# innnky/vispeech

Hardware: AMD Instinct MI355X
Metric: 44.1kHz samples/sec (higher is better)
Workload: dtype f32 (split-f16 MFMA, 3-term); 1 GPU; C3: 64 mixed zh/ja utterances (~5 s each) per GPU, 44.1 kHz, hop 512, phoneme/duration/F0/energy/noise supplied, random-init (synthetic) weights of configs/config.json; 2 batches in flight per GPU; utterances_per_gpu=64, global_batch=64, padded_frames=489, frames_padded=31296, frames_computed=28902, parallelism=shard1, generator=f16s, controls=all, batches_in_flight=2

## Files before the change

### include/vispeech_hip.h

```cpp
#ifndef VISPEECH_HIP_H
#define VISPEECH_HIP_H

#include <stdint.h>

#ifdef __cplusplus
extern "C" {
#endif

#define VSP_ABI_VERSION 7

enum {
  VSP_OK = 0,
  VSP_ERR_ARG = -1,
  VSP_ERR_STATE = -2,
  VSP_ERR_HIP = -3,
  VSP_ERR_KEY = -4,
  VSP_ERR_SHAPE = -5,
  VSP_ERR_WORKSPACE = -6,
  VSP_ERR_UNSUPPORTED = -7
};

#define VSP_MAX_LIST 8

typedef struct vsp_config {
// ... 91 lines not shown
int64_t vsp_flow_workspace_bytes(const vsp_ctx* ctx, int B, int Tf);
int vsp_flow_reverse(vsp_ctx* ctx, void* stream, int B, int Tf, const float* z_p, const float* g,
                     const int64_t* frame_lengths, float* z, void* workspace, int64_t workspace_bytes);
int64_t vsp_wn_layer_workspace_bytes(const vsp_ctx* ctx, int which, int B, int T);
int vsp_wn_layer(vsp_ctx* ctx, void* stream, int which, int layer, int B, int T, float* x, const float* g,
                 const int64_t* lengths, float* skip, int accumulate, void* workspace, int64_t workspace_bytes);
int64_t vsp_generator_workspace_bytes(const vsp_ctx* ctx, int B, int T);
int vsp_generator_kind(const vsp_ctx* ctx);
int vsp_generator(vsp_ctx* ctx, void* stream, int B, int T, const float* z, const float* g,
                  float* o, void* workspace, int64_t workspace_bytes);
int vsp_generator_ragged(vsp_ctx* ctx, void* stream, int B, int T, const float* z, const float* g,
                         const int64_t* lengths, float* o, void* workspace, int64_t workspace_bytes);

int vsp_generator_halo_frames(const vsp_ctx* ctx);
int vsp_generator_frame_dependence(const vsp_ctx* ctx, int* back, int* fwd);
int64_t vsp_generator_stream_workspace_bytes(const vsp_ctx* ctx, int B, int chunk_frames);
int vsp_generator_stream_chunk(vsp_ctx* ctx, void* stream, int B, int T, const float* z, const float* g, int f0, int f1,
                               float* o_chunk, void* workspace, int64_t workspace_bytes);

typedef struct vsp_stream_row {
  const float* z;
  int64_t z_channel_stride;
  const float* g;
  int32_t L, f0, f1;
} vsp_stream_row;
int vsp_stream_rows_plan(const vsp_ctx* ctx, int B, const vsp_stream_row* rows, int32_t* lo, int32_t* hi, int32_t* span_max);
int64_t vsp_generator_stream_rows_workspace_bytes(const vsp_ctx* ctx, int B, int chunk_frames);
int vsp_generator_stream_rows(vsp_ctx* ctx, void* stream, int B, const vsp_stream_row* rows, void* out, int64_t out_stride,
                              int pcm, void* workspace, int64_t workspace_bytes);

// ... 173 lines not shown
```

### vispeech_amd/_lib.py

```python
from __future__ import annotations

import ctypes as C
import os
from typing import Optional

_HERE = os.path.dirname(os.path.abspath(__file__))
LIB_PATH = os.environ.get("VSP_LIB_PATH") or os.path.join(_HERE, "lib", "libvispeech_hip.so")

VSP_MAX_LIST = 8
ABI_VERSION = 7
DTYPES = {"float32": 0, "float16": 1, "bfloat16": 2, "float64": 3}
PROF_GENERATOR, PROF_ATTENTION, PROF_FRAME = 0, 1, 2
FLAG_NONFINITE_LATENT, FLAG_NONFINITE_WAVE = 1, 2

ERRORS = {0: "VSP_OK", -1: "VSP_ERR_ARG", -2: "VSP_ERR_STATE", -3: "VSP_ERR_HIP", -4: "VSP_ERR_KEY",
          -5: "VSP_ERR_SHAPE", -6: "VSP_ERR_WORKSPACE", -7: "VSP_ERR_UNSUPPORTED"}


class VspConfig(C.Structure):
    _fields_ = [
        ("n_vocab", C.c_int32), ("inter_channels", C.c_int32), ("hidden_channels", C.c_int32),
        ("filter_channels", C.c_int32), ("n_heads", C.c_int32), ("n_layers", C.c_int32),
        ("kernel_size", C.c_int32), ("n_resblock_kernels", C.c_int32),
        ("resblock_kernel_sizes", C.c_int32 * VSP_MAX_LIST), ("n_resblock_dilations", C.c_int32),
# ... 89 lines not shown
    "vsp_set_isolated": (_I, [_P, _I]),
    "vsp_get_isolated": (_I, [_P]),
    "vsp_set_noise_seeds": (_I, [_P, C.POINTER(_U64), _I]),
    "vsp_set_row_controls": (_I, [_P, C.POINTER(VspRowControl), _I]),
    "vsp_encoder_workspace_bytes": (_I64, [_P, _I, _I]),
    "vsp_encoder": (_I, [_P, _P, _I, _I, _I, _P, _P, _P, _P, _I64]),
    "vsp_length_regulate": (_I, [_P, _P, _I, _I, _I, _I, _P, _P, _P]),
    "vsp_flow_workspace_bytes": (_I64, [_P, _I, _I]),
    "vsp_flow_reverse": (_I, [_P, _P, _I, _I, _P, _P, _P, _P, _P, _I64]),
    "vsp_generator_workspace_bytes": (_I64, [_P, _I, _I]),
    "vsp_generator": (_I, [_P, _P, _I, _I, _P, _P, _P, _P, _I64]),
    "vsp_generator_ragged": (_I, [_P, _P, _I, _I, _P, _P, _P, _P, _P, _I64]),
    "vsp_generator_kind": (_I, [_P]),
    "vsp_generator_halo_frames": (_I, [_P]),
    "vsp_generator_frame_dependence": (_I, [_P, C.POINTER(_I), C.POINTER(_I)]),
    "vsp_generator_stream_workspace_bytes": (_I64, [_P, _I, _I]),
    "vsp_generator_stream_chunk": (_I, [_P, _P, _I, _I, _P, _P, _I, _I, _P, _P, _I64]),
    "vsp_stream_rows_plan": (_I, [_P, _I, C.POINTER(VspStreamRow), C.POINTER(C.c_int32), C.POINTER(C.c_int32),
                                  C.POINTER(C.c_int32)]),
    "vsp_generator_stream_rows_workspace_bytes": (_I64, [_P, _I, _I]),
    "vsp_generator_stream_rows": (_I, [_P, _P, _I, C.POINTER(VspStreamRow), _P, _I64, _I, _P, _I64]),
    "vsp_stream_rows_output_plan": (_I, [_I, _I, _I, _I, _I, C.POINTER(VspStreamRow), C.POINTER(_I64), C.POINTER(_I64),
                                         C.POINTER(_I64), C.POINTER(_I64)]),
    "vsp_output_history_samples": (_I, [_I, _I, _I]),
    "vsp_stream_rows_out_samples": (_I64, [_I, _I, _I, _I, _I]),
    "vsp_generator_stream_rows_output": (_I, [_P, _P, _I, C.POINTER(VspStreamRowOut), _P, _I64, _I, _P, _I64]),
    "vsp_flow_forward": (_I, [_P, _P, _I, _I, _P, _P, _P, _P, _P, _I64]),
    "vsp_voice_conversion_workspace_bytes": (_I64, [_P, _I, _I]),
    "vsp_voice_conversion": (_I, [_P, _P, _I, _I, _P, _P, _P, _P, _P, _P, _P, _P, _P, _P, _P, _P, _P, _I64]),
    "vsp_posterior_workspace_bytes": (_I64, [_P, _I, _I]),
# ... 132 lines not shown
```

### vispeech_amd/csrc/api_common.h

```cpp
#pragma once
#include <algorithm>
#include <cmath>
#include <cstdlib>
#include <cstring>
#include <vector>

#include "model.h"
#include "row_controls.h"

namespace vsp {

struct T3 {
  float* p = nullptr;
  long bs = 0, cs = 0;
  T3 chan(int c) const { return T3{p ? p + (size_t)c * cs : nullptr, bs, cs}; }
};

struct Ws {
  char* base;
  size_t cap;
  size_t cur = 0;
  bool dry;
  bool overflow = false;
  Ws(void* b, size_t c, bool d) : base((char*)b), cap(c), dry(d) {}
// ... 202 lines not shown
  return ctx->fail(VSP_ERR_WORKSPACE, "%s workspace too small: %lld < %lld bytes", what, (long long)workspace_bytes, (long long)need);
}

int check_ready(vsp_ctx* ctx);
int check_vc(vsp_ctx* ctx);

void run_encoder_masked(Run& r, const EncoderW& E, int B, int T, T3 x_in, const int64_t* lengths, T3 y_out);
void mask3(Run& r, T3 x, const int64_t* lengths, int B, int C, int T);
void run_wn(Run& r, const Conv* cond, const std::vector<Conv>& in, const std::vector<Conv>& res, const std::vector<Conv>& skip,
            int nl, int B, int T, T3 H, T3 ACT, T3 OUT, float* gc, long gc_bs, const float* g, const int64_t* lengths);
void run_flow(Run& r, int B, int T, T3 z, const float* g, const int64_t* lengths, bool reverse = true);
void run_posterior(Run& r, int B, int T, T3 y, const int64_t* lengths, const float* g, const float* noise, T3 Z, T3 M, T3 LOGS,
                   float noise_scale = 1.f);
void draw_noise_rows(Run& r, uint64_t* seeds_dev, const int64_t* lengths, int B, int C, int T, float* drawn);
void run_gen(Run& r, int B, int T, T3 z, const int64_t* in_lengths, const float* g, float* o);

}
```

### vispeech_amd/csrc/api_context.hip

```cpp
#include "api_common.h"

using namespace vsp;

namespace vsp {

int check_ready(vsp_ctx* ctx) {
  if (!ctx) return VSP_ERR_ARG;
  if (!ctx->ready) return ctx->fail(VSP_ERR_STATE, "weights not finalised");
  return VSP_OK;
}

int check_vc(vsp_ctx* ctx) {
  const int rc = check_ready(ctx);
  if (rc) return rc;
  if (ctx->cfg.spec_channels <= 0) return ctx->fail(VSP_ERR_STATE, "context was created without spec_channels");
  if (!ctx->model.has_vc) return ctx->fail(VSP_ERR_STATE, "enc_q.* tensors were not loaded before vsp_finalize_weights");
  return VSP_OK;
}

}

extern "C" {

int vsp_abi_version(void) { return VSP_ABI_VERSION; }
// ... 11 lines not shown
  if (const char* e = getenv("VSP_ATT")) ctx->att_f16s = strcmp(e, "f32") != 0;
  bool want_f16 = false;
  if (const char* e = getenv("VSP_GENERATOR")) {
    if (!strcmp(e, "f32")) ctx->gen_mode = 0;
    want_f16 = !strcmp(e, "f16");
  }
  if (const char* e = getenv("VSP_FUSE_PAIRS")) ctx->fuse_pairs = atoi(e) != 0;
  if (const char* e = getenv("VSP_RB2_FUSE")) ctx->rb2_fuse = atoi(e) != 0;
  if (const char* e = getenv("VSP_TIMG")) ctx->t_img = atoi(e) != 0;
  if (const char* e = getenv("VSP_PP")) ctx->pp_pairs = atoi(e) != 0;
  if (const char* e = getenv("VSP_PAIR")) ctx->pair_ring = !strcmp(e, "ring");
  if (const char* e = getenv("VSP_CHAIN_RING")) ctx->chain_ring = atoi(e) != 0;
  if (const char* e = getenv("VSP_CHAIN")) ctx->chain_mask = atoi(e);
  if (const char* e = getenv("VSP_RW64")) ctx->rw64 = atoi(e) != 0;
  if (const char* e = getenv("VSP_TRIM_TAILS")) ctx->trim_tails = atoi(e) != 0;
  if (const char* e = getenv("VSP_COLS")) ctx->cols = atoi(e) != 0;
  if (const char* e = getenv("VSP_COLS_BLOCKS")) ctx->cols_blocks = atol(e);
  if (const char* e = getenv("VSP_COLS_MIN_BLOCKS")) ctx->cols_min_blocks = atol(e);
  if (const char* e = getenv("VSP_ACT_SCALE_LOG2")) {
    const int l = atoi(e);
    ctx->act_scale = std::ldexp(1.f, l < 0 ? 0 : l > 8 ? 8 : l);
  }
  if (const char* e = getenv("VSP_EARLY_FL")) ctx->early_fl = atoi(e) != 0;
  if (const char* e = getenv("VSP_RB_STREAMS")) ctx->rb_streams = atoi(e);
#ifdef VSP_EXPERIMENTS
  if (const char* e = getenv("VSP_ATT_KSPLIT")) ctx->att_ksplit = atoi(e);
  if (const char* e = getenv("VSP_CHUNK_MB")) ctx->chunk_mb = atof(e);
  if (const char* e = getenv("VSP_CHAIN_CH")) ctx->chain_ch = atoi(e);
  if (const char* e = getenv("VSP_CHAIN128")) ctx->chain128_mask = atoi(e);
#endif
// ... 2 lines not shown
  if (want_f16 && ctx->gen_mode == 1) ctx->gen_mode = 2;
  *out = ctx;
  return rc;
}

int vsp_destroy(vsp_ctx* ctx) {
  if (!ctx) return VSP_ERR_ARG;
  for (auto e : ctx->ev_pool) (void)hipEventDestroy(e);
  for (auto e : ctx->sync_ev) (void)hipEventDestroy(e);
  if (ctx->fl_ev) (void)hipEventDestroy(ctx->fl_ev);
  if (ctx->fl_pinned) (void)hipHostFree(ctx->fl_pinned);
  if (ctx->flags_host) (void)hipHostFree(ctx->flags_host);
  for (auto st : ctx->side) if (st) (void)hipStreamDestroy(st);
  if (ctx->arena && ctx->arena_owned) (void)hipFree(ctx->arena);
  if (ctx->out_tab) (void)hipFree(ctx->out_tab);
  for (auto& r : ctx->in_rates) if (r.tab) (void)hipFree(r.tab);
  for (auto& r : ctx->out_rates) if (r.tab) (void)hipFree(r.tab);
  delete ctx;
  return VSP_OK;
}

const char* vsp_last_error(const vsp_ctx* ctx) { return ctx ? ctx->err.c_str() : "null context"; }

int vsp_status(vsp_ctx* ctx, unsigned* flags, int clear) {
  if (!ctx || !flags) return VSP_ERR_ARG;
  *flags = 0u;
  if (!ctx->flags_host) return VSP_OK;
  volatile unsigned* w = ctx->flags_host;
  *flags = clear ? __atomic_exchange_n(ctx->flags_host, 0u, __ATOMIC_ACQ_REL) : *w;
  return VSP_OK;
}

int vsp_begin_weights(vsp_ctx* ctx) {
  if (!ctx) return VSP_ERR_ARG;
  ctx->raw.clear();
  ctx->ready = false;
  ctx->adopted_pending = false;
  return VSP_OK;
}

int vsp_set_weight(vsp_ctx* ctx, const char* key, const float* host_data, const int64_t* shape, int ndim) {
  if (!ctx || !key || !host_data || !shape || ndim < 0 || ndim > 8) return ctx ? ctx->fail(VSP_ERR_ARG, "null argument") : VSP_ERR_ARG;
  const std::string k(key);
  if (k.rfind("enc_q.", 0) == 0 && ctx->cfg.spec_channels <= 0) return VSP_OK;
  auto it = ctx->schema.find(k);
  bool folded_form = false;
  if (it == ctx->schema.end()) {
    auto iv = ctx->schema.find(k + "_v");
    if (iv == ctx->schema.end()) return ctx->fail(VSP_ERR_KEY, "unknown state_dict key '%s'", key);
    it = iv;
    folded_form = true;
  }
// ... 137 lines not shown

int vsp_finalize_weights(vsp_ctx* ctx, void* dev_arena) {
  if (!ctx) return VSP_ERR_ARG;
  if (ctx->model.total_floats == 0) return ctx->fail(VSP_ERR_STATE, "context was not planned (vsp_create failed)");
  const int miss = vsp_missing_weights(ctx);
  if (miss) return ctx->fail(VSP_ERR_STATE, "%d infer-path tensors missing", miss);
  std::vector<float> host;
  int rc = fill_model(ctx, host);
  if (rc) return rc;
  {
    const uint64_t tf = ctx->model.total_floats;
    const uint32_t hdr[6] = {ARENA_MAGIC, (uint32_t)VSP_ABI_VERSION, (uint32_t)(tf & 0xffffffffu), (uint32_t)(tf >> 32),
                             ctx->model.has_vc ? ARENA_FLAG_VC : 0u, config_hash(ctx)};
    std::memcpy(host.data(), hdr, sizeof hdr);
  }
  rc = set_arena(ctx, dev_arena);
  if (rc) return rc;
  hipError_t e = hipMemcpy(ctx->arena, host.data(), host.size() * sizeof(float), hipMemcpyHostToDevice);
  if (e != hipSuccess) return ctx->fail(VSP_ERR_HIP, "hipMemcpy(weight arena): %s", hipGetErrorString(e));
  ctx->adopted_pending = false;
  ctx->ready = true;
  return VSP_OK;
}

int vsp_adopt_packed_weights(vsp_ctx* ctx, void* dev_arena) {
  if (!ctx || !dev_arena) return ctx ? ctx->fail(VSP_ERR_ARG, "null arena") : VSP_ERR_ARG;
  if (ctx->model.total_floats == 0) return ctx->fail(VSP_ERR_STATE, "context was not planned");
  const int rc = set_arena(ctx, dev_arena);
  if (rc) return rc;
  ctx->model.has_vc = false;
  ctx->ready = false;
  ctx->adopted_pending = true;
  return VSP_OK;
}

int vsp_commit_adopted_weights(vsp_ctx* ctx, void* stream) {
  if (!ctx) return VSP_ERR_ARG;
  if (!ctx->adopted_pending || !ctx->arena) return ctx->fail(VSP_ERR_STATE, "no adopted arena to commit");
  uint32_t hdr[6] = {0, 0, 0, 0, 0, 0};
  hipError_t e = hipMemcpyAsync(hdr, ctx->arena, sizeof hdr, hipMemcpyDeviceToHost, (hipStream_t)stream);
  if (e == hipSuccess) e = hipStreamSynchronize((hipStream_t)stream);
  if (e != hipSuccess) return ctx->fail(VSP_ERR_HIP, "arena header read: %s", hipGetErrorString(e));
  const uint64_t tf = (uint64_t)hdr[2] | ((uint64_t)hdr[3] << 32);
  if (hdr[0] != ARENA_MAGIC) return ctx->fail(VSP_ERR_STATE, "adopted arena has no header (bytes not broadcast yet, or not a packed arena)");
  if (hdr[1] != (uint32_t)VSP_ABI_VERSION) return ctx->fail(VSP_ERR_STATE, "adopted arena was packed by ABI %u, this library is ABI %d", hdr[1], VSP_ABI_VERSION);
  if (tf != ctx->model.total_floats || hdr[5] != config_hash(ctx))
    return ctx->fail(VSP_ERR_STATE, "adopted arena was packed for a different configuration");
  ctx->model.has_vc = (hdr[4] & ARENA_FLAG_VC) != 0;
  ctx->adopted_pending = false;
  ctx->ready = true;
  return VSP_OK;
}

int vsp_has_voice_conversion(const vsp_ctx* ctx) { return ctx && ctx->ready && ctx->model.has_vc ? 1 : 0; }

int vsp_weight_arena(const vsp_ctx* ctx, void** dev_arena, int64_t* bytes) {
  if (!ctx || !dev_arena || !bytes) return VSP_ERR_ARG;
  *dev_arena = ctx->arena;
  *bytes = (int64_t)(ctx->model.total_floats * sizeof(float));
  return VSP_OK;
}

int vsp_randn(void* stream, uint64_t seed, int64_t n, float* out) { return vsp_randn_at(stream, seed, 0, n, out); }

int vsp_randn_at(void* stream, uint64_t seed, int64_t first, int64_t n, float* out) {
// ... 193 lines not shown
```

### vispeech_amd/csrc/api_generator.hip

```cpp
#include "api_common.h"

using namespace vsp;

namespace {

inline int64_t r256(int64_t n) { return (n + 255) / 256 * 256; }

long resblock_support(const vsp_config& c, int resblock, int j) {
  const long kk = c.resblock_kernel_sizes[j];
  long acc = 0;
  if (resblock == 2) {
    for (int d = 0; d < 2 && d < c.n_resblock_dilations; ++d) acc += (kk - 1) * c.resblock_dilation_sizes[j][d] / 2;
    return acc;
  }
  for (int d = 0; d < c.n_resblock_dilations; ++d) acc += (kk - 1) * c.resblock_dilation_sizes[j][d] / 2 + (kk - 1) / 2;
  return acc;
}

void generator_frame_dependence(const vsp_config& c, int resblock, int pre_k, int post_k, int& back, int& fwd) {
  long lo = -(pre_k - 1) / 2, hi = (pre_k - 1) / 2, up = 1;
  for (int i = 0; i < c.n_upsamples; ++i) {
    const long s = c.upsample_rates[i], k = c.upsample_kernel_sizes[i], p = (k - s) / 2;
    lo = lo * s - p; hi = hi * s - p + k - 1; up *= s;
    long rb = 0;
    for (int j = 0; j < c.n_resblock_kernels; ++j) rb = std::max(rb, resblock_support(c, resblock, j));
    lo -= rb; hi += rb;
  }
  lo -= (post_k - 1) / 2; hi += (post_k - 1) / 2;
  back = (int)(hi / up);
  fwd = (int)((up - 1 - lo) / up);
}

long total_upsample(const vsp_config& c) {
  long u = 1;
  for (int i = 0; i < c.n_upsamples; ++i) u *= c.upsample_rates[i];
  return u;
}

template <class F>
size_t max_over_stages(const vsp_config& c, int T, size_t mx, F f) {
  long t = T;
  for (int i = 0; i < c.n_upsamples; ++i) {
    t *= c.upsample_rates[i];
    mx = std::max(mx, (size_t)f(c.upsample_initial_channel >> (i + 1), t));
  }
  return mx;
}

void run_generator(Run& r, int B, int T, T3 z, const int64_t* in_lengths, const float* g, float* o) {
  const vsp_config& c = r.ctx->cfg;
  const Model& m = r.ctx->model;
// ... 168 lines not shown
  std::vector<float*> side_buf;
  if (r.ctx->rb_streams)
    for (int j = 1; j < nk; ++j)
      for (int u = 0; u < 2; ++u) side_buf.push_back(r.ws.f((size_t)B * mx));
  const size_t mx_img = max_over_stages(
      c, T, 0, [&](int ch, long t) { return cl_stage_img(*r.ctx, ch) ? cl_img_halfs(ch, (int)t) / 2 : (size_t)0; });
  const bool want_img = mx_img != 0;
  uint16_t* timg = want_img ? reinterpret_cast<uint16_t*>(r.ws.f((size_t)B * mx_img)) : nullptr;
  std::vector<uint16_t*> side_img;
  if (want_img && r.ctx->rb_streams)
    for (int j = 1; j < nk; ++j) side_img.push_back(reinterpret_cast<uint16_t*>(r.ws.f((size_t)B * mx_img)));
  int back = 0, fwd = 0;
  generator_frame_dependence(c, r.ctx->resblock, m.g_pre.K, m.post_k, back, fwd);
  const bool iso = r.iso && in_lengths;
  int* glen_all = reinterpret_cast<int*>(r.ws.bytes((size_t)B * sizeof(int)));
  bool trim = in_lengths && (iso || (r.ctx->trim_tails && T > back + fwd + 1 &&
                                                 (size_t)fwd * total_upsample(c) * sizeof(float) <= 64 * 1024));
  if (trim && r.host_lengths) {
    bool any = false;
    for (int b = 0; b < B; ++b) any = any || std::max<int64_t>(r.host_lengths[b], 0) + (iso ? 0 : back + 1 + fwd) < T;
    trim = any;
  }
  if (trim && !r.dry() && r.ok())
    r.chk(iso ? launch_gen_plan_isolated(in_lengths, B, T, glen_all, r.s) : launch_gen_plan(in_lengths, B, T, back, fwd, glen_all, r.s),
          "gen_plan");
  std::vector<int> glen_host;
  if (trim && r.ctx->prof_on && !r.dry() && r.ok()) {
    glen_host.resize(B);
    hipError_t e = hipMemcpyAsync(glen_host.data(), glen_all, (size_t)B * sizeof(int), hipMemcpyDeviceToHost, r.s);
    if (e == hipSuccess) e = hipStreamSynchronize(r.s);
    r.chk(e, "gen_plan read-back (profiling)");
  }
  if (mx * sizeof(float) >= (size_t)1 << 31 || (timg && mx_img * sizeof(float) >= (size_t)1 << 31)) {
    if (r.rc == VSP_OK)
      r.rc = r.ctx->fail(VSP_ERR_UNSUPPORTED, "generator: %d frames per call exceed the 2 GiB per-utterance activation "
                                              "limit; synthesise in chunks (Engine.generator_stream)", T);
    return;
  }
  ConvArgs a = r.args(m.g_pre, z, X0, T, T);
  a.lengths = in_lengths; a.in_mask = in_lengths ? 1 : 0;
  a.cond = gc; a.cond_bs = c0;
  r.conv(a, B, true);
  int cur = 0;
  if (!r.dry() && r.ok())
// ... 7 lines not shown
    ch = c0 >> (i + 1);
    int fb[4], nf = 0;
    for (int k = 0; k < 5; ++k) if (k != cur) fb[nf++] = k;
    float *XU = buf[fb[0]], *T1 = buf[fb[1]], *YA = buf[fb[2]], *XS = buf[fb[3]];
    const long bs = Tout * ch, xbs = Tn * cin;
    int Bc = B;
    if (r.ctx->chunk_mb > 0) {
      const double per_utt_mb = (double)bs * 4.0 / (1024.0 * 1024.0);
      Bc = (int)std::max(1.0, std::floor(r.ctx->chunk_mb / per_utt_mb));
      const long tiles_per_utt = (Tout + 255) / 256 * std::max(1, ch / 128);
      const int min_b = (int)((2 * 256 * (ch >= 128 ? 1 : 2) + tiles_per_utt - 1) / tiles_per_utt);
      Bc = std::min(B, std::max(Bc, min_b));
    }
    for (int b0 = 0; b0 < B; b0 += Bc) {
      const int nb = std::min(Bc, B - b0);
      r.glen = trim ? glen_all + b0 : nullptr;
      r.grate_in = (int)(Tn / T); r.grate_out = (int)(Tout / T);
      r.work_frac = 1.0;
      if (!glen_host.empty() && r.ok()) {
        double fr = 0.0;
        for (int b = b0; b < b0 + nb; ++b) fr += glen_host[b];
        r.work_frac = fr / ((double)nb * T);
      }
      const float* xin = buf[cur] + (size_t)b0 * xbs;
      float *xu = XU + (size_t)b0 * bs, *xs = XS + (size_t)b0 * bs;
      r.clconv(U, xin, xu, nullptr, (int)Tn, false, 1.f, nb);
      const bool conc = ((r.ctx->rb_streams >> i) & 1) && !r.ctx->prof_on && !r.dry() && r.ok() && Bc == B && nk > 1 &&
                        (int)side_buf.size() == 2 * (nk - 1) && ensure_side_streams(r, (size_t)c.n_upsamples * (nk + 1));
      hipStream_t const main_s = r.s;
      hipEvent_t* const ev = conc ? r.ctx->sync_ev.data() + (size_t)i * (nk + 1) : nullptr;
      const bool use_img = timg && cl_stage_img(*r.ctx, ch);
      auto chain_img = [&](int j) -> uint16_t* {
        if (!use_img) return nullptr;
        uint16_t* base = (conc && j != 1 && (int)side_img.size() == nk - 1) ? side_img[j == 0 ? 0 : j - 1] : timg;
        return base + (size_t)b0 * cl_img_halfs(ch, (int)Tout);
      };
// ... 29 lines not shown
          else r.clfused(rb, ch, u.p0, u.np, u.kind == RbLaunch::Pair, yin, yout, (int)Tout, acc, div, nb);
          yin = yout;
        }
        if (conc) r.chk(hipEventRecord(ev[1 + j], r.s), "chain end event");
        r.s = main_s;
      }
      if (conc) r.chk(hipStreamWaitEvent(main_s, ev[nk], 0), "join wait");
    }
    cur = fb[3];
    Tn = Tout;
  }
  r.glen = nullptr;
  r.work_frac = 1.0;
  if (!r.dry() && r.ok()) {
    r.chk(launch_conv_post_cl(buf[cur], Tn * ch, ch, r.A(m.post_wt), m.post_c, m.post_k, 0.01f, o, Tn, B, (int)Tn, r.s,
                              trim ? glen_all : nullptr, (int)(Tn / T), 1.f / r.ctx->act_scale, r.ctx->flags_dev), "conv_post_cl");
    if (trim && iso) r.chk(launch_gen_tail_zero(o, Tn, in_lengths, B, T, (int)(Tn / T), r.s), "gen_tail_zero");
    else if (trim) r.chk(launch_gen_tail_fill(o, Tn, in_lengths, glen_all, B, T, back, fwd, (int)(Tn / T), r.s), "gen_tail_fill");
  }
}

}

namespace vsp {

void run_gen(Run& r, int B, int T, T3 z, const int64_t* in_lengths, const float* g, float* o) {
  if (r.ctx->gen_mode >= 1 && r.ctx->model.has_cl) run_generator_cl(r, B, T, z, in_lengths, g, o);
  else run_generator(r, B, T, z, in_lengths, g, o);
}

}

extern "C" {

int64_t vsp_generator_workspace_bytes(const vsp_ctx* ctx, int B, int T) {
  if (!ctx || B <= 0 || T <= 0) return VSP_ERR_ARG;
  return dry_bytes(ctx, [&](Run& r) { run_gen(r, B, T, T3{}, nullptr, nullptr, nullptr); });
}

int vsp_generator(vsp_ctx* ctx, void* stream, int B, int T, const float* z, const float* g, float* o, void* workspace,
                  int64_t workspace_bytes) {
  int rc = check_ready(ctx);
  if (rc) return rc;
// ... 25 lines not shown
  long w = 3;
  for (int i = c.n_upsamples - 1; i >= 0; --i) {
    long rb = 0;
    for (int j = 0; j < c.n_resblock_kernels; ++j) rb = std::max(rb, resblock_support(c, ctx->resblock, j));
    w += rb;
    const int s = c.upsample_rates[i], k = c.upsample_kernel_sizes[i];
    w = (w + (k + s) / 2 - 1 + s - 1) / s;
  }
  return (int)(w + 3);
}

int vsp_generator_frame_dependence(const vsp_ctx* ctx, int* back, int* fwd) {
  if (!ctx || !back || !fwd) return VSP_ERR_ARG;
  generator_frame_dependence(ctx->cfg, ctx->resblock, ctx->model.g_pre.K > 0 ? ctx->model.g_pre.K : 7, ctx->model.post_k,
                             *back, *fwd);
  return VSP_OK;
}

int64_t vsp_generator_stream_workspace_bytes(const vsp_ctx* ctx, int B, int chunk_frames) {
  if (!ctx || B <= 0 || chunk_frames <= 0) return VSP_ERR_ARG;
  const int span = chunk_frames + 2 * vsp_generator_halo_frames(ctx);
  const int64_t g = vsp_generator_workspace_bytes(ctx, B, span);
  if (g < 0) return g;
  return g + r256((int64_t)B * span * total_upsample(ctx->cfg) * (int64_t)sizeof(float));
}

int vsp_generator_stream_chunk(vsp_ctx* ctx, void* stream, int B, int T, const float* z, const float* g, int f0, int f1,
                               float* o_chunk, void* workspace, int64_t workspace_bytes) {
  int rc = check_ready(ctx);
  if (rc) return rc;
// ... 159 lines not shown
```

### vispeech_amd/csrc/cl_misc.hip

```cpp
#include "kernels.h"

namespace vsp {

typedef unsigned u32x4 __attribute__((ext_vector_type(4)));

__global__ void __launch_bounds__(256) transpose_ct_kernel(const float* __restrict__ x, long x_bs, long x_cs,
                                                           float* __restrict__ y, long y_bs, int y_ts, int C, int T,
                                                           float scale) {
  __shared__ float tile[32][33];
  const int b = blockIdx.z, c0 = blockIdx.y * 32, t0 = blockIdx.x * 32;
  const int lx = threadIdx.x & 31, ly = threadIdx.x >> 5;
#pragma unroll
  for (int k = 0; k < 4; ++k) {
    const int c = c0 + ly + 8 * k, t = t0 + lx;
    tile[ly + 8 * k][lx] = (c < C && t < T) ? x[(size_t)b * x_bs + (size_t)c * x_cs + t] : 0.f;
  }
  __syncthreads();
#pragma unroll
  for (int k = 0; k < 4; ++k) {
    const int t = t0 + ly + 8 * k, c = c0 + lx;
    if (t < T && c < C) y[(size_t)b * y_bs + (size_t)t * y_ts + c] = tile[lx][ly + 8 * k] * scale;
  }
}
hipError_t launch_transpose_ct(const float* x, long x_bs, long x_cs, float* y, long y_bs, int y_ts, int B, int C,
// ... 74 lines not shown
    T = glen[blockIdx.x / planes_per_utt] * grate;
    end = CL_IMG_PADF + T + CL_IMG_PADB;
  }
  for (int r = threadIdx.x; r < CL_IMG_PADF; r += 256) pl[r] = z;
  for (int r = CL_IMG_PADF + T + threadIdx.x; r < end; r += 256) pl[r] = z;
}
hipError_t launch_cl_img_zero_pads(uint16_t* img, int B, int C, int T, hipStream_t s, const int* glen, int grate) {
  if (B <= 0 || C % 32 || T <= 0 || (reinterpret_cast<uintptr_t>(img) & 15)) return hipErrorInvalidValue;
  const int ppu = (C / 32) * 8;
  const long planes = (long)B * ppu;
  hipLaunchKernelGGL(cl_img_zero_pads_kernel, dim3((unsigned)planes), dim3(256), 0, s, reinterpret_cast<uint4*>(img), T,
                     cl_img_tpad(T), ppu, glen, grate);
  return hipGetLastError();
}

__global__ void gen_plan_kernel(const int64_t* __restrict__ lengths, int B, int T, int ext, int* __restrict__ glen) {
  const int b = blockIdx.x * blockDim.x + threadIdx.x;
  if (b >= B) return;
  long len = lengths[b];
  len = len < 0 ? 0 : len;
  const long e = len + ext;
  glen[b] = e < T ? (int)e : T;
}
hipError_t launch_gen_plan(const int64_t* lengths, int B, int T, int back, int fwd, int* glen, hipStream_t s) {
  if (!lengths || !glen || B <= 0 || T <= 0 || back < 0 || fwd < 0) return hipErrorInvalidValue;
  hipLaunchKernelGGL(gen_plan_kernel, dim3((B + 63) / 64), dim3(64), 0, s, lengths, B, T, back + 1 + fwd, glen);
  return hipGetLastError();
}
__global__ void __launch_bounds__(1024) gen_tail_fill_kernel(float* __restrict__ o, long o_bs, const int64_t* __restrict__ lengths,
                                                             const int* __restrict__ glen, int T, int back, int fwd, int up) {
  extern __shared__ float tail[];
  const int b = blockIdx.x;
  if (glen[b] >= T) return;
  long len = lengths[b];
  len = len < 0 ? 0 : len;
  float* ob = o + (size_t)b * o_bs;
  const long s0 = (len + back) * up;
  const long e0 = s0 + up;
  const int nt = fwd * up;
  for (int i = threadIdx.x; i < nt; i += blockDim.x) tail[i] = ob[e0 + i];
  __syncthreads();
  const long fill_end = (long)(T - fwd) * up;
  for (long i = e0 + threadIdx.x; i < fill_end; i += blockDim.x) ob[i] = ob[s0 + (i - e0) % up];
  for (int i = threadIdx.x; i < nt; i += blockDim.x) ob[fill_end + i] = tail[i];
}
hipError_t launch_gen_tail_fill(float* o, long o_bs, const int64_t* lengths, const int* glen, int B, int T, int back, int fwd,
                                int up, hipStream_t s) {
  if (!o || !lengths || !glen || B <= 0 || T <= 0 || back < 0 || fwd < 0 || up <= 0) return hipErrorInvalidValue;
  const size_t lds = (size_t)fwd * up * sizeof(float);
  if (lds > 64 * 1024) return hipErrorInvalidValue;
  hipLaunchKernelGGL(gen_tail_fill_kernel, dim3(B), dim3(1024), lds, s, o, o_bs, lengths, glen, T, back, fwd, up);
  return hipGetLastError();
}

__global__ void gen_plan_isolated_kernel(const int64_t* __restrict__ lengths, int B, int T, int* __restrict__ glen) {
  const int b = blockIdx.x * blockDim.x + threadIdx.x;
  if (b >= B) return;
  const long len = lengths[b];
  glen[b] = len < 1 ? 1 : (len < T ? (int)len : T);
}
hipError_t launch_gen_plan_isolated(const int64_t* lengths, int B, int T, int* glen, hipStream_t s) {
  if (!lengths || !glen || B <= 0 || T <= 0) return hipErrorInvalidValue;
  hipLaunchKernelGGL(gen_plan_isolated_kernel, dim3((B + 63) / 64), dim3(64), 0, s, lengths, B, T, glen);
  return hipGetLastError();
}
__global__ void __launch_bounds__(256) gen_tail_zero_kernel(float* __restrict__ o, long o_bs, const int64_t* __restrict__ lengths,
// ... 24 lines not shown
```

### vispeech_amd/csrc/kernels.h

```cpp
#pragma once
#include <hip/hip_runtime.h>
#include <stdint.h>

#include <atomic>

#include "../../include/vispeech_hip.h"

namespace vsp {

inline hipError_t set_max_dynamic_lds(const void* kern, int bytes, std::atomic<uint64_t>& done) {
  int dev = 0;
  hipError_t e = hipGetDevice(&dev);
  if (e != hipSuccess) return e;
  const uint64_t bit = 1ull << (dev & 63);
  if (done.load(std::memory_order_acquire) & bit) return hipSuccess;
  e = hipFuncSetAttribute(kern, hipFuncAttributeMaxDynamicSharedMemorySize, bytes);
  if (e == hipSuccess) done.fetch_or(bit, std::memory_order_release);
  return e;
}

constexpr int CONV_CK = 32;
constexpr int CONV_HALO = 64;

struct ConvArgs {
// ... 165 lines not shown
hipError_t launch_g16_rw64(const ClPairArgs& a, int B, hipStream_t s);
bool g16_pp_supported(int C, int K, int dil, int terms);
hipError_t launch_g16_pp(const ClPairArgs& a, int B, hipStream_t s);
size_t packed_g16_halfs(int rows, int Cin, int K);
void pack_g16_weights(uint16_t* dst, int rows, int Cin, int K, const float* dense );
inline size_t ups_weight_offset(int ci, int co, int r, int tap, int Cout, int s, int kt) {
  return ((size_t)ci * Cout + co) * ((size_t)kt * s) + (size_t)s * (kt - 1 - tap) + r;
}
hipError_t launch_spec_to_mel(const float* spec, const float* basis, const int* lo, const int* hi, float* mel, int B,
                              int n_freq, int n_mels, int T, hipStream_t s);
hipError_t launch_transpose_ct(const float* x, long x_bs, long x_cs, float* y, long y_bs, int y_ts, int B, int C,
                               int T, hipStream_t s, float scale = 1.f);
hipError_t launch_conv_post_cl(const float* x, long x_bs, int x_ts, const float* w, int C, int K, float slope,
                               float* o, long o_bs, int B, int T, hipStream_t s, const int* glen = nullptr, int grate = 0,
                               float unscale = 1.f, unsigned* flags = nullptr);
hipError_t launch_gen_plan(const int64_t* lengths, int B, int T, int back, int fwd, int* glen, hipStream_t s);
hipError_t launch_gen_tail_fill(float* o, long o_bs, const int64_t* lengths, const int* glen, int B, int T, int back, int fwd,
                                int up, hipStream_t s);
hipError_t launch_gen_plan_isolated(const int64_t* lengths, int B, int T, int* glen, hipStream_t s);
hipError_t launch_gen_tail_zero(float* o, long o_bs, const int64_t* lengths, int B, int T, int up, hipStream_t s);

hipError_t launch_attention(const float* qkv, long qkv_bs, long qkv_cs, const float* emb_k,
                            const float* emb_v, const int64_t* lengths, float* out, long o_bs,
                            long o_cs, int B, int H, int n_heads, int T, int window, int ksplit_mode, hipStream_t s);

size_t attn_pack_bytes(int B, int n_heads, int DK, int T);
hipError_t launch_attention_f16s(const float* qkv, long qkv_bs, long qkv_cs, const float* emb_k, const float* emb_v,
                                 const int64_t* lengths, float* out, long o_bs, long o_cs, int B, int H, int n_heads, int T,
                                 int window, void* workspace, hipStream_t s, int block_mode = -1);
bool attn_qkv_pack_supported(int H, int n_heads);
hipError_t launch_attn_qkv_pack_f16s(const float* x, long x_bs, long x_cs, const uint16_t* wg, const float* bias,
                                     const int64_t* lengths, int B, int H, int n_heads, int T, void* workspace, hipStream_t s);

// ... 159 lines not shown
```

### vispeech_amd/csrc/model.h

```cpp
#pragma once
#include <hip/hip_runtime.h>

#include <cstdarg>
#include <cstdio>
#include <map>
#include <string>
#include <vector>

#include "../../include/vispeech_hip.h"
#include "kernels.h"

namespace vsp {

struct HostTensor {
  std::vector<int64_t> shape;
  std::vector<float> data;
  size_t numel() const { size_t n = 1; for (auto s : shape) n *= (size_t)s; return n; }
};

struct Conv {
  int M = 0, Cin = 0, K = 1, dil = 1, pad = 0;
  int ups_s = 0, ups_p = 0;
  size_t w = 0;
  long b = -1;
// ... 83 lines not shown
  float* arena = nullptr;
  bool arena_owned = false;
  bool ready = false;
  bool t_img = true;
  bool pp_pairs = true;
  bool pair_ring = false;
  bool chain_ring = false;
  bool rw64 = false;
  float act_scale = 16.f;
  unsigned* flags_host = nullptr;
  unsigned* flags_dev = nullptr;
  long cols_min_blocks = 32;
  long cols_blocks = 256;
  bool cols = true;
  bool trim_tails = true;
  int rb_streams = 0;
  bool early_fl = true;
  int64_t* fl_pinned = nullptr;
  int fl_cap = 0, fl_n = 0;
  hipEvent_t fl_ev = nullptr;
  const int64_t* fl_src = nullptr;
  std::vector<int64_t> fl_known;
  const int64_t* fl_known_src = nullptr;
  hipStream_t side[2] = {nullptr, nullptr};
  std::vector<hipEvent_t> sync_ev;
  float* out_tab = nullptr;
  int out_L = 0, out_M = 0, out_H = 0, out_J = 0, out_P = 0;
  struct InputRate { int rate = 0; float* tab = nullptr; int L = 0, M = 0, H = 0, J = 0, P = 0; };
  InputRate in_rates[VSP_INPUT_RATES_MAX];
  InputRate out_rates[VSP_OUTPUT_RATES_MAX];
// ... 45 lines not shown
```

### vispeech_amd/engine.py

```python
from __future__ import annotations

import ctypes as C
from typing import Dict, Mapping, Optional, Sequence

import numpy as np
import torch

from . import _lib
from .schema import ModelDims


def _ptr(t: Optional[torch.Tensor]):
    return None if t is None else C.c_void_p(t.data_ptr())


def _dev_f32(t, device) -> torch.Tensor:
    return torch.as_tensor(t).to(device=device, dtype=torch.float32).contiguous()


def _dev_i64(t, device) -> torch.Tensor:
    return torch.as_tensor(t).to(device=device, dtype=torch.int64).contiguous()


class OutputHistory:
# ... 628 lines not shown
        return o

    @property
    def generator_kind(self) -> int:
        return int(self.lib.vsp_generator_kind(self.ctx))

    @property
    def generator_halo(self) -> int:
        return int(self.lib.vsp_generator_halo_frames(self.ctx))

    def generator_frame_dependence(self):
        b, f = C.c_int(), C.c_int()
        _lib.check(self.lib.vsp_generator_frame_dependence(self.ctx, C.byref(b), C.byref(f)), self.ctx,
                   "vsp_generator_frame_dependence")
        return int(b.value), int(f.value)

    def generator_stream(self, z, g, chunk_frames: int = 256):
        z = _dev_f32(z, self.device)
        g = _dev_f32(g, self.device).reshape(z.shape[0], -1)
        B, _, T = z.shape
        up = self.dims.total_upsample
        ws = self._workspace("generator_stream", self.lib.vsp_generator_stream_workspace_bytes(self.ctx, B, chunk_frames))
        for f0 in range(0, T, chunk_frames):
            f1 = min(T, f0 + chunk_frames)
            o = self._f(B, 1, (f1 - f0) * up)
            with torch.cuda.device(self.device):
                rc = self.lib.vsp_generator_stream_chunk(self.ctx, self._stream(), B, T, _ptr(z), _ptr(g), f0, f1,
                                                         _ptr(o), _ptr(ws), ws.numel())
            _lib.check(rc, self.ctx, "vsp_generator_stream_chunk")
            yield o
# ... 383 lines not shown
```

Baseline: 205.4 million samples/s.

## Precompute per-speaker generator tail table to trim padded frames in later stages

When weights are loaded, the generator is run once on a zero latent for every speaker embedding, and the resulting steady-state tail waveform is stored in a table. At inference, a small kernel matches each row's conditioning vector to a speaker row. For matched rows, the upsample stages after the first compute fewer padded frames (reach1 instead of fwd+1), and the tail is filled from the table. This removes redundant generator work in the padded region, at the cost of extra memory, a slower weight load, a per-batch matching kernel, and reliance on zero padding beyond each row's length.

```diff
diff --git a/include/vispeech_hip.h b/include/vispeech_hip.h
--- a/include/vispeech_hip.h
+++ b/include/vispeech_hip.h
@@ -129,6 +129,7 @@
 
 int vsp_generator_halo_frames(const vsp_ctx* ctx);
 int vsp_generator_frame_dependence(const vsp_ctx* ctx, int* back, int* fwd);
+int vsp_generator_tail_extents(const vsp_ctx* ctx, int* back, int* fwd, int* reach1);
 int64_t vsp_generator_stream_workspace_bytes(const vsp_ctx* ctx, int B, int chunk_frames);
 int vsp_generator_stream_chunk(vsp_ctx* ctx, void* stream, int B, int T, const float* z, const float* g, int f0, int f1,
                                float* o_chunk, void* workspace, int64_t workspace_bytes);
diff --git a/vispeech_amd/_lib.py b/vispeech_amd/_lib.py
--- a/vispeech_amd/_lib.py
+++ b/vispeech_amd/_lib.py
@@ -127,6 +127,7 @@
     "vsp_generator_kind": (_I, [_P]),
     "vsp_generator_halo_frames": (_I, [_P]),
     "vsp_generator_frame_dependence": (_I, [_P, C.POINTER(_I), C.POINTER(_I)]),
+    "vsp_generator_tail_extents": (_I, [_P, C.POINTER(_I), C.POINTER(_I), C.POINTER(_I)]),
     "vsp_generator_stream_workspace_bytes": (_I64, [_P, _I, _I]),
     "vsp_generator_stream_chunk": (_I, [_P, _P, _I, _I, _P, _P, _I, _I, _P, _P, _I64]),
     "vsp_stream_rows_plan": (_I, [_P, _I, C.POINTER(VspStreamRow), C.POINTER(C.c_int32), C.POINTER(C.c_int32),
diff --git a/vispeech_amd/csrc/api_common.h b/vispeech_amd/csrc/api_common.h
--- a/vispeech_amd/csrc/api_common.h
+++ b/vispeech_amd/csrc/api_common.h
@@ -240,5 +240,7 @@
                    float noise_scale = 1.f);
 void draw_noise_rows(Run& r, uint64_t* seeds_dev, const int64_t* lengths, int B, int C, int T, float* drawn);
 void run_gen(Run& r, int B, int T, T3 z, const int64_t* in_lengths, const float* g, float* o);
+void tail_table_build(vsp_ctx* ctx, hipStream_t s);
+void tail_table_drop(vsp_ctx* ctx);
 
 }
diff --git a/vispeech_amd/csrc/api_context.hip b/vispeech_amd/csrc/api_context.hip
--- a/vispeech_amd/csrc/api_context.hip
+++ b/vispeech_amd/csrc/api_context.hip
@@ -49,6 +49,7 @@
   if (const char* e = getenv("VSP_CHAIN")) ctx->chain_mask = atoi(e);
   if (const char* e = getenv("VSP_RW64")) ctx->rw64 = atoi(e) != 0;
   if (const char* e = getenv("VSP_TRIM_TAILS")) ctx->trim_tails = atoi(e) != 0;
+  if (const char* e = getenv("VSP_TAIL_TABLE")) ctx->tail_table_on = atoi(e) != 0;
   if (const char* e = getenv("VSP_COLS")) ctx->cols = atoi(e) != 0;
   if (const char* e = getenv("VSP_COLS_BLOCKS")) ctx->cols_blocks = atol(e);
   if (const char* e = getenv("VSP_COLS_MIN_BLOCKS")) ctx->cols_min_blocks = atol(e);
@@ -81,6 +82,7 @@
   for (auto st : ctx->side) if (st) (void)hipStreamDestroy(st);
   if (ctx->arena && ctx->arena_owned) (void)hipFree(ctx->arena);
   if (ctx->out_tab) (void)hipFree(ctx->out_tab);
+  tail_table_drop(ctx);
   for (auto& r : ctx->in_rates) if (r.tab) (void)hipFree(r.tab);
   for (auto& r : ctx->out_rates) if (r.tab) (void)hipFree(r.tab);
   delete ctx;
@@ -103,6 +105,7 @@
   ctx->raw.clear();
   ctx->ready = false;
   ctx->adopted_pending = false;
+  tail_table_drop(ctx);
   return VSP_OK;
 }
 
@@ -270,18 +273,21 @@
                              ctx->model.has_vc ? ARENA_FLAG_VC : 0u, config_hash(ctx)};
     std::memcpy(host.data(), hdr, sizeof hdr);
   }
+  tail_table_drop(ctx);
   rc = set_arena(ctx, dev_arena);
   if (rc) return rc;
   hipError_t e = hipMemcpy(ctx->arena, host.data(), host.size() * sizeof(float), hipMemcpyHostToDevice);
   if (e != hipSuccess) return ctx->fail(VSP_ERR_HIP, "hipMemcpy(weight arena): %s", hipGetErrorString(e));
   ctx->adopted_pending = false;
   ctx->ready = true;
+  tail_table_build(ctx, nullptr);
   return VSP_OK;
 }
 
 int vsp_adopt_packed_weights(vsp_ctx* ctx, void* dev_arena) {
   if (!ctx || !dev_arena) return ctx ? ctx->fail(VSP_ERR_ARG, "null arena") : VSP_ERR_ARG;
   if (ctx->model.total_floats == 0) return ctx->fail(VSP_ERR_STATE, "context was not planned");
+  tail_table_drop(ctx);
   const int rc = set_arena(ctx, dev_arena);
   if (rc) return rc;
   ctx->model.has_vc = false;
@@ -305,6 +311,7 @@
   ctx->model.has_vc = (hdr[4] & ARENA_FLAG_VC) != 0;
   ctx->adopted_pending = false;
   ctx->ready = true;
+  tail_table_build(ctx, (hipStream_t)stream);
   return VSP_OK;
 }
 
diff --git a/vispeech_amd/csrc/api_generator.hip b/vispeech_amd/csrc/api_generator.hip
--- a/vispeech_amd/csrc/api_generator.hip
+++ b/vispeech_amd/csrc/api_generator.hip
@@ -17,24 +17,43 @@
   return acc;
 }
 
-void generator_frame_dependence(const vsp_config& c, int resblock, int pre_k, int post_k, int& back, int& fwd) {
-  long lo = -(pre_k - 1) / 2, hi = (pre_k - 1) / 2, up = 1;
-  for (int i = 0; i < c.n_upsamples; ++i) {
+void generator_support(const vsp_config& c, int resblock, int pre_k, int post_k, int first, int end, long& lo, long& hi, long& up) {
+  lo = hi = 0; up = 1;
+  if (first == 0) { lo = -(pre_k - 1) / 2; hi = (pre_k - 1) / 2; }
+  for (int i = first; i < end && i < c.n_upsamples; ++i) {
     const long s = c.upsample_rates[i], k = c.upsample_kernel_sizes[i], p = (k - s) / 2;
     lo = lo * s - p; hi = hi * s - p + k - 1; up *= s;
     long rb = 0;
     for (int j = 0; j < c.n_resblock_kernels; ++j) rb = std::max(rb, resblock_support(c, resblock, j));
     lo -= rb; hi += rb;
   }
-  lo -= (post_k - 1) / 2; hi += (post_k - 1) / 2;
-  back = (int)(hi / up);
-  fwd = (int)((up - 1 - lo) / up);
+  if (end >= c.n_upsamples) { lo -= (post_k - 1) / 2; hi += (post_k - 1) / 2; }
 }
 
 long total_upsample(const vsp_config& c) {
   long u = 1;
   for (int i = 0; i < c.n_upsamples; ++i) u *= c.upsample_rates[i];
   return u;
+}
+
+void generator_frame_dependence(const vsp_config& c, int resblock, int pre_k, int post_k, int& back, int& fwd) {
+  long lo, hi, up;
+  generator_support(c, resblock, pre_k, post_k, 0, c.n_upsamples, lo, hi, up);
+  back = (int)(hi / up);
+  fwd = (int)((up - 1 - lo) / up);
+}
+
+void generator_tail_reach(const vsp_config& c, int resblock, int pre_k, int post_k, int& reach1, int& fwd0) {
+  int back = 0, fwd = 0;
+  generator_frame_dependence(c, resblock, pre_k, post_k, back, fwd);
+  reach1 = fwd + 1; fwd0 = fwd;
+  if (c.n_upsamples < 2) return;
+  const long total = total_upsample(c);
+  long lo, hi, up;
+  generator_support(c, resblock, pre_k, post_k, 1, c.n_upsamples, lo, hi, up);
+  reach1 = std::max(1, (int)((total - 1 - lo) / total));
+  generator_support(c, resblock, pre_k, post_k, 0, 1, lo, hi, up);
+  fwd0 = (int)((up - 1 - lo) / up);
 }
 
 template <class F>
@@ -233,6 +252,8 @@
   generator_frame_dependence(c, r.ctx->resblock, m.g_pre.K, m.post_k, back, fwd);
   const bool iso = r.iso && in_lengths;
   int* glen_all = reinterpret_cast<int*>(r.ws.bytes((size_t)B * sizeof(int)));
+  int* glen1_all = reinterpret_cast<int*>(r.ws.bytes((size_t)B * sizeof(int)));
+  int* tail_row = reinterpret_cast<int*>(r.ws.bytes((size_t)B * sizeof(int)));
   bool trim = in_lengths && (iso || (r.ctx->trim_tails && T > back + fwd + 1 &&
                                                  (size_t)fwd * total_upsample(c) * sizeof(float) <= 64 * 1024));
   if (trim && r.host_lengths) {
@@ -240,13 +261,23 @@
     for (int b = 0; b < B; ++b) any = any || std::max<int64_t>(r.host_lengths[b], 0) + (iso ? 0 : back + 1 + fwd) < T;
     trim = any;
   }
-  if (trim && !r.dry() && r.ok())
-    r.chk(iso ? launch_gen_plan_isolated(in_lengths, B, T, glen_all, r.s) : launch_gen_plan(in_lengths, B, T, back, fwd, glen_all, r.s),
+  const float* const table = r.ctx->tail_table;
+  const bool tabled = trim && !iso && table && r.ctx->tail_back == back && r.ctx->tail_fwd == fwd;
+  const int* glen1 = tabled ? glen1_all : glen_all;
+  if (trim && !r.dry() && r.ok()) {
+    if (tabled)
+      r.chk(launch_gen_tail_rows(g, r.A(m.emb_g), c.n_speakers, c.gin_channels, B, tail_row, r.s), "gen_tail_rows");
+    r.chk(iso ? launch_gen_plan_isolated(in_lengths, B, T, glen_all, r.s)
+              : launch_gen_plan(in_lengths, B, T, back, fwd, tabled ? r.ctx->tail_reach1 : fwd + 1, tabled ? tail_row : nullptr,
+                                glen_all, glen1_all, r.s),
           "gen_plan");
-  std::vector<int> glen_host;
+  }
+  std::vector<int> glen_host, glen1_host;
   if (trim && r.ctx->prof_on && !r.dry() && r.ok()) {
     glen_host.resize(B);
+    glen1_host.resize(B);
     hipError_t e = hipMemcpyAsync(glen_host.data(), glen_all, (size_t)B * sizeof(int), hipMemcpyDeviceToHost, r.s);
+    if (e == hipSuccess) e = hipMemcpyAsync(glen1_host.data(), glen1, (size_t)B * sizeof(int), hipMemcpyDeviceToHost, r.s);
     if (e == hipSuccess) e = hipStreamSynchronize(r.s);
     r.chk(e, "gen_plan read-back (profiling)");
   }
@@ -284,12 +315,13 @@
     }
     for (int b0 = 0; b0 < B; b0 += Bc) {
       const int nb = std::min(Bc, B - b0);
-      r.glen = trim ? glen_all + b0 : nullptr;
+      r.glen = trim ? (i == 0 ? glen_all : glen1) + b0 : nullptr;
       r.grate_in = (int)(Tn / T); r.grate_out = (int)(Tout / T);
       r.work_frac = 1.0;
       if (!glen_host.empty() && r.ok()) {
+        const std::vector<int>& gh = i == 0 ? glen_host : glen1_host;
         double fr = 0.0;
-        for (int b = b0; b < b0 + nb; ++b) fr += glen_host[b];
+        for (int b = b0; b < b0 + nb; ++b) fr += gh[b];
         r.work_frac = fr / ((double)nb * T);
       }
       const float* xin = buf[cur] + (size_t)b0 * xbs;
@@ -349,9 +381,11 @@
   r.work_frac = 1.0;
   if (!r.dry() && r.ok()) {
     r.chk(launch_conv_post_cl(buf[cur], Tn * ch, ch, r.A(m.post_wt), m.post_c, m.post_k, 0.01f, o, Tn, B, (int)Tn, r.s,
-                              trim ? glen_all : nullptr, (int)(Tn / T), 1.f / r.ctx->act_scale, r.ctx->flags_dev), "conv_post_cl");
+                              trim ? glen1 : nullptr, (int)(Tn / T), 1.f / r.ctx->act_scale, r.ctx->flags_dev), "conv_post_cl");
     if (trim && iso) r.chk(launch_gen_tail_zero(o, Tn, in_lengths, B, T, (int)(Tn / T), r.s), "gen_tail_zero");
-    else if (trim) r.chk(launch_gen_tail_fill(o, Tn, in_lengths, glen_all, B, T, back, fwd, (int)(Tn / T), r.s), "gen_tail_fill");
+    else if (trim)
+      r.chk(launch_gen_tail_fill(o, Tn, in_lengths, glen_all, glen1, tabled ? tail_row : nullptr, table, B, T, back, fwd, (int)(Tn / T),
+                                 r.s), "gen_tail_fill");
   }
 }
 
@@ -362,6 +396,70 @@
 void run_gen(Run& r, int B, int T, T3 z, const int64_t* in_lengths, const float* g, float* o) {
   if (r.ctx->gen_mode >= 1 && r.ctx->model.has_cl) run_generator_cl(r, B, T, z, in_lengths, g, o);
   else run_generator(r, B, T, z, in_lengths, g, o);
+}
+
+void tail_table_drop(vsp_ctx* ctx) {
+  if (ctx->tail_table) (void)hipFree(ctx->tail_table);
+  ctx->tail_table = nullptr;
+}
+
+void tail_table_build(vsp_ctx* ctx, hipStream_t s) {
+  constexpr int TAIL_BUILD_B = 64;
+  tail_table_drop(ctx);
+  const vsp_config& c = ctx->cfg;
+  const Model& m = ctx->model;
+  if (!ctx->tail_table_on || !ctx->trim_tails || ctx->gen_mode != 1 || !m.has_cl || !ctx->arena) return;
+  if (c.n_speakers < 1 || c.n_speakers > 4096) return;
+  int back = 0, fwd = 0, reach1 = 0, fwd0 = 0;
+  generator_frame_dependence(c, ctx->resblock, m.g_pre.K, m.post_k, back, fwd);
+  generator_tail_reach(c, ctx->resblock, m.g_pre.K, m.post_k, reach1, fwd0);
+  const long up = total_upsample(c);
+  if ((size_t)fwd * up * sizeof(float) > 64 * 1024) return;
+  if (reach1 >= fwd + 1 || fwd0 + reach1 > fwd + 1) return;
+  const int T = back + 1 + fwd, Bc = std::min(c.n_speakers, TAIL_BUILD_B);
+  const size_t row = (size_t)(1 + fwd) * up;
+  const int64_t gen = dry_bytes(ctx, [&](Run& r) { run_gen(r, Bc, T, T3{}, nullptr, nullptr, nullptr); });
+  if (gen < 0) return;
+  const size_t z_bytes = (size_t)r256((int64_t)Bc * c.inter_channels * T * (int64_t)sizeof(float));
+  const size_t o_bytes = (size_t)r256((int64_t)Bc * T * up * (int64_t)sizeof(float));
+  char* scratch = nullptr;
+  float* table = nullptr;
+  hipError_t e = hipMalloc(reinterpret_cast<void**>(&table), (size_t)c.n_speakers * row * sizeof(float));
+  if (e == hipSuccess) e = hipMalloc(reinterpret_cast<void**>(&scratch), z_bytes + o_bytes + (size_t)gen);
+  if (e == hipSuccess) e = hipMemsetAsync(scratch, 0, z_bytes, s);
+  const bool prof_on = ctx->prof_on;
+  unsigned* const flags_dev = ctx->flags_dev;
+  const std::string err = ctx->err;
+  ctx->prof_on = false;
+  ctx->flags_dev = nullptr;
+  int rc = VSP_OK;
+  for (int s0 = 0; s0 < c.n_speakers && e == hipSuccess && rc == VSP_OK; s0 += Bc) {
+    const int nb = std::min(Bc, c.n_speakers - s0);
+    float* const z = reinterpret_cast<float*>(scratch);
+    float* const o = reinterpret_cast<float*>(scratch + z_bytes);
+    Ws ws(scratch + z_bytes + o_bytes, (size_t)gen, false);
+    Run r{ctx, s, ws};
+    run_gen(r, nb, T, ext(z, c.inter_channels, T), nullptr, ctx->arena + m.emb_g + (size_t)s0 * c.gin_channels, o);
+    rc = ws.overflow ? VSP_ERR_WORKSPACE : r.rc;
+    if (rc == VSP_OK)
+      e = hipMemcpy2DAsync(table + (size_t)s0 * row, row * sizeof(float), o + (size_t)back * up, (size_t)T * up * sizeof(float),
+                           row * sizeof(float), (size_t)nb, hipMemcpyDeviceToDevice, s);
+  }
+  ctx->prof_on = prof_on;
+  ctx->flags_dev = flags_dev;
+  ctx->err = err;
+  if (scratch || table) {
+    const hipError_t es = hipStreamSynchronize(s);
+    if (e == hipSuccess) e = es;
+  }
+  if (scratch) (void)hipFree(scratch);
+  if (e != hipSuccess || rc != VSP_OK) {
+    if (table) (void)hipFree(table);
+    (void)hipGetLastError();
+    return;
+  }
+  ctx->tail_table = table;
+  ctx->tail_back = back; ctx->tail_fwd = fwd; ctx->tail_reach1 = reach1;
 }
 
 }
@@ -417,6 +515,15 @@
   if (!ctx || !back || !fwd) return VSP_ERR_ARG;
   generator_frame_dependence(ctx->cfg, ctx->resblock, ctx->model.g_pre.K > 0 ? ctx->model.g_pre.K : 7, ctx->model.post_k,
                              *back, *fwd);
+  return VSP_OK;
+}
+
+int vsp_generator_tail_extents(const vsp_ctx* ctx, int* back, int* fwd, int* reach1) {
+  if (!ctx || !back || !fwd || !reach1) return VSP_ERR_ARG;
+  const int pre_k = ctx->model.g_pre.K > 0 ? ctx->model.g_pre.K : 7;
+  int fwd0 = 0;
+  generator_frame_dependence(ctx->cfg, ctx->resblock, pre_k, ctx->model.post_k, *back, *fwd);
+  generator_tail_reach(ctx->cfg, ctx->resblock, pre_k, ctx->model.post_k, *reach1, fwd0);
   return VSP_OK;
 }
 
diff --git a/vispeech_amd/csrc/cl_misc.hip b/vispeech_amd/csrc/cl_misc.hip
--- a/vispeech_amd/csrc/cl_misc.hip
+++ b/vispeech_amd/csrc/cl_misc.hip
@@ -112,42 +112,83 @@
   return hipGetLastError();
 }
 
-__global__ void gen_plan_kernel(const int64_t* __restrict__ lengths, int B, int T, int ext, int* __restrict__ glen) {
+__global__ void __launch_bounds__(256) gen_tail_rows_kernel(const unsigned* __restrict__ g, const unsigned* __restrict__ emb_g,
+                                                            int n_speakers, int gin, int* __restrict__ tail_row) {
+  __shared__ int best;
+  const int b = blockIdx.x;
+  if (threadIdx.x == 0) best = 0x7fffffff;
+  __syncthreads();
+  const unsigned* gb = g + (size_t)b * gin;
+  for (int s = threadIdx.x; s < n_speakers; s += blockDim.x) {
+    const unsigned* row = emb_g + (size_t)s * gin;
+    int i = 0;
+    while (i < gin && row[i] == gb[i]) ++i;
+    if (i == gin) { atomicMin(&best, s); break; }
+  }
+  __syncthreads();
+  if (threadIdx.x == 0) tail_row[b] = best == 0x7fffffff ? -1 : best;
+}
+hipError_t launch_gen_tail_rows(const float* g, const float* emb_g, int n_speakers, int gin, int B, int* tail_row, hipStream_t s) {
+  if (!g || !emb_g || !tail_row || n_speakers <= 0 || gin <= 0 || B <= 0) return hipErrorInvalidValue;
+  hipLaunchKernelGGL(gen_tail_rows_kernel, dim3(B), dim3(256), 0, s, reinterpret_cast<const unsigned*>(g),
+                     reinterpret_cast<const unsigned*>(emb_g), n_speakers, gin, tail_row);
+  return hipGetLastError();
+}
+__global__ void gen_plan_kernel(const int64_t* __restrict__ lengths, int B, int T, int back, int fwd, int reach1,
+                                const int* __restrict__ tail_row, int* __restrict__ glen0, int* __restrict__ glen1) {
   const int b = blockIdx.x * blockDim.x + threadIdx.x;
   if (b >= B) return;
   long len = lengths[b];
   len = len < 0 ? 0 : len;
-  const long e = len + ext;
-  glen[b] = e < T ? (int)e : T;
-}
-hipError_t launch_gen_plan(const int64_t* lengths, int B, int T, int back, int fwd, int* glen, hipStream_t s) {
-  if (!lengths || !glen || B <= 0 || T <= 0 || back < 0 || fwd < 0) return hipErrorInvalidValue;
-  hipLaunchKernelGGL(gen_plan_kernel, dim3((B + 63) / 64), dim3(64), 0, s, lengths, B, T, back + 1 + fwd, glen);
+  const long e = len + back + 1 + fwd;
+  const int e0 = e < T ? (int)e : T;
+  int e1 = e0;
+  if (tail_row && tail_row[b] >= 0 && len + back + fwd <= T) {
+    const long e1l = len + back + reach1;
+    e1 = e1l < e0 ? (int)e1l : e0;
+  }
+  glen0[b] = e0;
+  glen1[b] = e1;
+}
+hipError_t launch_gen_plan(const int64_t* lengths, int B, int T, int back, int fwd, int reach1, const int* tail_row, int* glen0,
+                           int* glen1, hipStream_t s) {
+  if (!lengths || !glen0 || !glen1 || B <= 0 || T <= 0 || back < 0 || fwd < 0 || reach1 < 1) return hipErrorInvalidValue;
+  hipLaunchKernelGGL(gen_plan_kernel, dim3((B + 63) / 64), dim3(64), 0, s, lengths, B, T, back, fwd, reach1, tail_row, glen0, glen1);
   return hipGetLastError();
 }
 __global__ void __launch_bounds__(1024) gen_tail_fill_kernel(float* __restrict__ o, long o_bs, const int64_t* __restrict__ lengths,
-                                                             const int* __restrict__ glen, int T, int back, int fwd, int up) {
+                                                             const int* __restrict__ glen0, const int* __restrict__ glen1,
+                                                             const int* __restrict__ tail_row, const float* __restrict__ table,
+                                                             int T, int back, int fwd, int up) {
   extern __shared__ float tail[];
   const int b = blockIdx.x;
-  if (glen[b] >= T) return;
+  const int g0 = glen0[b], g1 = glen1[b];
   long len = lengths[b];
   len = len < 0 ? 0 : len;
   float* ob = o + (size_t)b * o_bs;
   const long s0 = (len + back) * up;
+  const long fill_end = (long)(T - fwd) * up;
+  const int nt = fwd * up;
+  if (g1 < g0) {
+    const float* row = table + (size_t)tail_row[b] * (size_t)(1 + fwd) * up;
+    for (long i = s0 + threadIdx.x; i < fill_end; i += blockDim.x) ob[i] = row[(i - s0) % up];
+    for (int i = threadIdx.x; i < nt; i += blockDim.x) ob[fill_end + i] = row[up + i];
+    return;
+  }
+  if (g0 >= T) return;
   const long e0 = s0 + up;
-  const int nt = fwd * up;
   for (int i = threadIdx.x; i < nt; i += blockDim.x) tail[i] = ob[e0 + i];
   __syncthreads();
-  const long fill_end = (long)(T - fwd) * up;
   for (long i = e0 + threadIdx.x; i < fill_end; i += blockDim.x) ob[i] = ob[s0 + (i - e0) % up];
   for (int i = threadIdx.x; i < nt; i += blockDim.x) ob[fill_end + i] = tail[i];
 }
-hipError_t launch_gen_tail_fill(float* o, long o_bs, const int64_t* lengths, const int* glen, int B, int T, int back, int fwd,
-                                int up, hipStream_t s) {
-  if (!o || !lengths || !glen || B <= 0 || T <= 0 || back < 0 || fwd < 0 || up <= 0) return hipErrorInvalidValue;
+hipError_t launch_gen_tail_fill(float* o, long o_bs, const int64_t* lengths, const int* glen0, const int* glen1, const int* tail_row,
+                                const float* table, int B, int T, int back, int fwd, int up, hipStream_t s) {
+  if (!o || !lengths || !glen0 || !glen1 || B <= 0 || T <= 0 || back < 0 || fwd < 0 || up <= 0) return hipErrorInvalidValue;
   const size_t lds = (size_t)fwd * up * sizeof(float);
   if (lds > 64 * 1024) return hipErrorInvalidValue;
-  hipLaunchKernelGGL(gen_tail_fill_kernel, dim3(B), dim3(1024), lds, s, o, o_bs, lengths, glen, T, back, fwd, up);
+  hipLaunchKernelGGL(gen_tail_fill_kernel, dim3(B), dim3(1024), lds, s, o, o_bs, lengths, glen0, glen1, tail_row, table, T, back, fwd,
+                     up);
   return hipGetLastError();
 }
 
diff --git a/vispeech_amd/csrc/kernels.h b/vispeech_amd/csrc/kernels.h
--- a/vispeech_amd/csrc/kernels.h
+++ b/vispeech_amd/csrc/kernels.h
@@ -203,9 +203,11 @@
 hipError_t launch_conv_post_cl(const float* x, long x_bs, int x_ts, const float* w, int C, int K, float slope,
                                float* o, long o_bs, int B, int T, hipStream_t s, const int* glen = nullptr, int grate = 0,
                                float unscale = 1.f, unsigned* flags = nullptr);
-hipError_t launch_gen_plan(const int64_t* lengths, int B, int T, int back, int fwd, int* glen, hipStream_t s);
-hipError_t launch_gen_tail_fill(float* o, long o_bs, const int64_t* lengths, const int* glen, int B, int T, int back, int fwd,
-                                int up, hipStream_t s);
+hipError_t launch_gen_tail_rows(const float* g, const float* emb_g, int n_speakers, int gin, int B, int* tail_row, hipStream_t s);
+hipError_t launch_gen_plan(const int64_t* lengths, int B, int T, int back, int fwd, int reach1, const int* tail_row, int* glen0,
+                           int* glen1, hipStream_t s);
+hipError_t launch_gen_tail_fill(float* o, long o_bs, const int64_t* lengths, const int* glen0, const int* glen1, const int* tail_row,
+                                const float* table, int B, int T, int back, int fwd, int up, hipStream_t s);
 hipError_t launch_gen_plan_isolated(const int64_t* lengths, int B, int T, int* glen, hipStream_t s);
 hipError_t launch_gen_tail_zero(float* o, long o_bs, const int64_t* lengths, int B, int T, int up, hipStream_t s);
 
diff --git a/vispeech_amd/csrc/model.h b/vispeech_amd/csrc/model.h
--- a/vispeech_amd/csrc/model.h
+++ b/vispeech_amd/csrc/model.h
@@ -121,6 +121,9 @@
   long cols_blocks = 256;
   bool cols = true;
   bool trim_tails = true;
+  bool tail_table_on = true;
+  float* tail_table = nullptr;
+  int tail_back = 0, tail_fwd = 0, tail_reach1 = 0;
   int rb_streams = 0;
   bool early_fl = true;
   int64_t* fl_pinned = nullptr;
diff --git a/vispeech_amd/engine.py b/vispeech_amd/engine.py
--- a/vispeech_amd/engine.py
+++ b/vispeech_amd/engine.py
@@ -666,6 +666,12 @@
         _lib.check(self.lib.vsp_generator_frame_dependence(self.ctx, C.byref(b), C.byref(f)), self.ctx,
                    "vsp_generator_frame_dependence")
         return int(b.value), int(f.value)
+
+    def generator_tail_extents(self):
+        b, f, r = C.c_int(), C.c_int(), C.c_int()
+        _lib.check(self.lib.vsp_generator_tail_extents(self.ctx, C.byref(b), C.byref(f), C.byref(r)), self.ctx,
+                   "vsp_generator_tail_extents")
+        return int(b.value), int(f.value), int(r.value)
 
     def generator_stream(self, z, g, chunk_frames: int = 256):
         z = _dev_f32(z, self.device)
```

Result: faster. 208.8 million samples/s (median of 6 runs) (+1.6%).
